# google-deepmind/dm_control

Measured on AMD Instinct MI355X. Metric: env-steps/s (whole node) at batch 4096; max rel qpos error vs CPU, higher is better.
Workload: dtype f32

## Files before the change

dm_control_amd/batch.py:

```python
import ctypes

import numpy as np

from dm_control_amd import _native
from dm_control_amd import mjcf_compiler

OUT = dict(sensor=1 << 0, xpos=1 << 1, xquat=1 << 2, xmat=1 << 3, xipos=1 << 4,
           geom=1 << 5, site=1 << 6, subtree_com=1 << 7, qacc=1 << 8,
           actuator=1 << 9, contact=1 << 10, qfrc=1 << 11, cvel=1 << 12, contact_ids=1 << 13)
OUT_ALL = 0x7fffffff


class BatchedPhysics:

  def __init__(self, model, batch_size, device_id=0, precision=32, nconmax=0,
               njmax=0, lanes_per_env=0, njcon=0, specialise=None):
    if not isinstance(model, mjcf_compiler.Model):
      raise TypeError('model must be a compiled mjcf_compiler.Model')
    L = _native.lib()
    self.model = model
    self.model_real = {}
    self.batch_size = int(batch_size)
    self.precision = precision
    self.device_id = device_id
# ... 34 lines not shown
  def set_task_args(self, blob):
    buf = (ctypes.c_char * len(blob)).from_buffer_copy(blob)
    _native.check(_native.lib().dmc_batch_set_task_args(self._ptr, ctypes.cast(buf, ctypes.c_void_p), len(blob)))

  def enable_task(self, on):
    _native.check(_native.lib().dmc_batch_enable_task(self._ptr, int(bool(on))))

  def close(self):
    L = _native.lib()
    if getattr(self, '_ptr', None):
      L.dmc_batch_destroy(self._ptr)
      self._ptr = None
    if getattr(self, '_model_ptr', None):
      L.dmc_model_destroy(self._model_ptr)
      self._model_ptr = None

  def __del__(self):
    try:
      self.close()
    except Exception:
      pass

  def info(self):
    a = np.zeros(21, dtype=np.int32)
    _native.check(_native.lib().dmc_batch_info(self._ptr, a.ctypes.data))
    keys = ['B', 'precision', 'lanes_per_env', 'waves_per_block', 'envs_per_block',
            'lds_bytes_per_block', 'grid', 'nconmax', 'njmax', 'env_scratch_bytes', 'static_id',
            'jac_kmax', 'table_lds_bytes', 'envs_per_cu', 'njdense', 'njcon', 'stash', 'stash_bytes_per_env',
            'global_scratch_bytes_per_env', 'work_queue', 'slices']
    return dict(zip(keys, (int(x) for x in a)))

  def _rows(self, name):
    rows, is_int = ctypes.c_int(), ctypes.c_int()
    _native.check(_native.lib().dmc_batch_field_rows(self._ptr, name.encode(),
                                                     ctypes.byref(rows), ctypes.byref(is_int)))
    return rows.value, bool(is_int.value)

  def get(self, name):
    rows, is_int = self._rows(name)
    if is_int:
      out = np.zeros((self.batch_size, rows), dtype=np.int32)
      _native.check(_native.lib().dmc_batch_get_int(self._ptr, name.encode(), out.ctypes.data))
    else:
      out = np.zeros((self.batch_size, rows), dtype=np.float64)
      if rows:
        _native.check(_native.lib().dmc_batch_get(self._ptr, name.encode(), out.ctypes.data))
    return out

  def set(self, name, value):
    rows, is_int = self._rows(name)
    if not rows:
      return
    dt = np.int32 if is_int else np.float64
# ... 213 lines not shown
```

dm_control_amd/csrc/dmc_api.hip:

```cpp
#include <hip/hip_runtime.h>
#include <dlfcn.h>

#include <cstdio>
#include <cstdlib>
#include <cstring>
#include <algorithm>
#include <string>
#include <type_traits>
#include <vector>

#include "../../include/dmc_batch.h"
#include "step_kernel.hip.h"
#include "step_tables.h"

namespace dmc {
hipError_t launch_step_f32(const LaunchGeom& g, hipStream_t stream, const StepLayout* d_layout, const StepOpts<float>& o,
                           const int* g_mi, const float* g_mr, const int* g_mc, const StepIO<float>& io, int nstep, int legacy, int mode, int outmask, int nsub);
hipError_t launch_step_f64(const LaunchGeom& g, hipStream_t stream, const StepLayout* d_layout, const StepOpts<double>& o,
                           const int* g_mi, const double* g_mr, const int* g_mc, const StepIO<double>& io, int nstep, int legacy, int mode, int outmask, int nsub);
}

using namespace dmc;

static thread_local std::string g_err;
static int fail(const std::string& msg, int code = -1) { g_err = msg; return code; }
#define HIP_TRY(expr)                                                                        \
  do {                                                                                       \
    hipError_t e_ = (expr);                                                                  \
    if (e_ != hipSuccess) return fail(std::string(#expr) + ": " + hipGetErrorString(e_), -2); \
  } while (0)

struct dmc_model {
  HostModel hm;
};

enum FieldId {
#define X(name, count, flags) F_##name,
  DMC_DATA_REAL_FIELDS(X) DMC_DATA_INT_FIELDS(X)
#undef X
  F_env_geom, F_COUNT
};
struct Field {
// ... 35 lines not shown
  int launched_mask = 0;
  int ndebug = 0;
  void* d_debug = nullptr;
  int* d_debug_i = nullptr;
  long long* d_prof = nullptr;
  size_t elem = 0;
  void* d_stash_r = nullptr; int* d_stash_i = nullptr; int* d_epoch = nullptr; int stash_on = 0; int stash_auto = 0;
  int xfrc_on = 0;
  void* d_ns_A = nullptr;
  int* d_work = nullptr;
  int ncu = 0;
  void* d_kstash = nullptr; int* d_kstash_i = nullptr;
  int *d_cost = nullptr, *d_order = nullptr; int lpt = 0, nitems = 0;
  int* d_prog = nullptr; int max_slices = 0;
  unsigned long long* d_hand = nullptr; int hand_n = 0; int nxcd = 1;
  void* d_gscr = nullptr;
  int* d_trace = nullptr;
  Profiler* prof = nullptr;
  Xfer* xfer = nullptr;
  void* d_probe = nullptr; int probe_geom = 0, probe_cap = 0;
  int trace_launch = 0;
  int* d_rj_i = nullptr; double* d_rj_r = nullptr;
  int* d_eg_slot = nullptr;
  void* spec_so = nullptr; void* spec_launch = nullptr; int spec_features = 0;
  int spec_task_bytes = 0;
  void* d_task_args = nullptr; int task_on = 0;
};

template <class Owner, typename P>
static int dev_alloc(Owner* b, P** ptr, size_t bytes, bool zero, const char* what, const void* init = nullptr) {
  void* p = nullptr;
  hipError_t e = hipMalloc(&p, bytes);
  if (e == hipSuccess && zero) e = hipMemset(p, 0, bytes);
  if (e == hipSuccess && init) e = hipMemcpy(p, init, bytes, hipMemcpyHostToDevice);
  if (e != hipSuccess) { if (p) (void)hipFree(p); return fail(std::string("hipMalloc") + (*what ? " " : "") + what + ": " + hipGetErrorString(e), -2); }
  b->dev_bufs.push_back(p);
  *ptr = (P*)p;
  return 0;
}
template <class Owner, typename P>
static void dev_free(Owner* b, P** ptr) {
  if (!*ptr) return;
  b->dev_bufs.erase(std::find(b->dev_bufs.begin(), b->dev_bufs.end(), (void*)*ptr));
  (void)hipFree(*ptr);
  *ptr = nullptr;
}
template <class Owner>
// ... 330 lines not shown
  if (!b || !so_path) return fail("null argument");
  void* h = dlopen(so_path, RTLD_NOW | RTLD_LOCAL);
  if (!h) return fail(std::string("cannot load ") + so_path + ": " + dlerror());
  typedef const StepLayout* (*layout_t)();
  typedef void (*info_t)(int*);
  layout_t fl = (layout_t)dlsym(h, "dmc_spec_layout");
  info_t fi = (info_t)dlsym(h, "dmc_spec_info");
  void* launch = dlsym(h, "dmc_spec_launch");
  if (!fl || !fi || !launch) { dlclose(h); return fail("not a specialisation plugin (dmc_spec_* symbols missing)"); }
  int info[8]; fi(info);
  if (info[4] != b->precision) { dlclose(h); return fail("the plugin was built for another precision"); }
  const int so = b->precision == 64 ? (int)sizeof(StepOpts<double>) : (int)sizeof(StepOpts<float>);
  const int sio = b->precision == 64 ? (int)sizeof(StepIO<double>) : (int)sizeof(StepIO<float>);
  if (info[0] != (int)sizeof(StepLayout) || info[1] != so || info[2] != sio || info[3] != DMC_MODEL_VERSION || info[7] != (int)sizeof(LaunchGeom)) {
    dlclose(h); return fail("the plugin was built from other sources than this library (struct sizes / model version differ)");
  }
  if (info[5] != b->geom.lpe) { dlclose(h); return fail("the plugin was built for another lanes-per-environment shape"); }
  if (memcmp(fl(), &b->tb.L, sizeof(StepLayout)) != 0) { dlclose(h); return fail("the plugin's layout is not this batch's (another model or other caps)"); }
  if (b->spec_so) dlclose(b->spec_so);
  b->spec_so = h; b->spec_launch = launch; b->spec_features = info[6];
  typedef int (*tb_t)();
  tb_t tb = (tb_t)dlsym(h, "dmc_spec_task_args_bytes");
  b->spec_task_bytes = tb ? tb() : 0;
  b->task_on = 0;
  return bump_epoch(b, 0, true);
}

extern "C" int dmc_batch_set_task_args(dmc_batch* b, const void* args, int nbytes) {
  if (!b || !args) return fail("null argument");
  if (!b->spec_task_bytes) return fail("the batch's kernel carries no task epilogue (attach a plugin built with a task header)");
  if (nbytes != b->spec_task_bytes) return fail("task argument block: size differs from the one the kernel was generated with");
  HIP_TRY(hipSetDevice(b->device));
  if (!b->d_task_args && dev_alloc(b, &b->d_task_args, (size_t)nbytes, false, "task arguments")) return -2;
  HIP_TRY(hipMemcpy(b->d_task_args, args, (size_t)nbytes, hipMemcpyHostToDevice));
  return 0;
}
extern "C" int dmc_batch_enable_task(dmc_batch* b, int on) {
  if (!b) return fail("null batch");
  if (on && (!b->spec_task_bytes || !b->d_task_args)) return fail("no task epilogue to enable (dmc_batch_set_task_args first)");
  b->task_on = on ? 1 : 0;
  return 0;
}

extern "C" int dmc_batch_step(dmc_batch* b, int nstep, int legacy_step, void* hip_stream) {
  if (!b) return fail("null batch");
  if (nstep < 1) return fail("nstep must be >= 1");
// ... 549 lines not shown
    if (reset_real(F_mocap_pos, mp.data(), 3*m.nmocap)) return -2;
    if (reset_real(F_mocap_quat, mq.data(), 4*m.nmocap)) return -2;
  }
  Field* w = &b->fields[F_warning];
  std::vector<int32_t> wh((size_t)B * DMC_NWARNING, 0);
  if (env_mask) { if (get_int(b, w, wh.data())) return -2; for (int e = 0; e < B; e++) if (env_mask[e]) for (int k = 0; k < DMC_NWARNING; k++) wh[(size_t)e * DMC_NWARNING + k] = 0; }
  return set_int(b, w, wh.data());
}

extern "C" int dmc_batch_info(const dmc_batch* b, int* info) {
  if (!b || !info) return fail("null argument");
  const StepLayout& L = b->tb.L;
  info[0] = b->B; info[1] = b->precision; info[2] = b->geom.lpe; info[3] = b->geom.waves; info[4] = b->geom.envs_per_block;
  info[5] = b->geom.lds_bytes; info[6] = b->geom.grid; info[7] = L.d.nconmax; info[8] = L.d.njmax;
  info[9] = (int)((size_t)L.n_sr * b->elem + (size_t)L.n_si * sizeof(int));
  info[10] = b->spec_launch ? 1000 : b->geom.static_id;
  info[11] = L.d.kmax;
  info[12] = b->geom.lds_bytes - b->geom.envs_per_block * info[9];
  { long blocks = (160L * 1024) / b->geom.lds_bytes; if (blocks * b->geom.waves > 8) blocks = 8 / b->geom.waves; info[13] = (int)(blocks * b->geom.envs_per_block); }
  info[14] = L.d.njdense; info[15] = L.d.njcon; info[16] = b->stash_on; info[17] = (int)((size_t)L.n_keep * b->elem + (size_t)(L.n_si + 4) * sizeof(int));
  info[18] = (int)((size_t)L.n_gs * b->elem);
  info[19] = b->geom.queue;
  info[20] = b->geom.queue ? b->max_slices : 0;
  return 0;
}

extern "C" int dmc_batch_enable_profiling(dmc_batch* b, int enabled) {
  if (!b) return fail("null batch");
  if (!b->prof) b->prof = new Profiler();
  b->prof->on = enabled != 0;
  return 0;
}
extern "C" int dmc_batch_get_timer(dmc_batch* b, int timer, double* duration_s, long long* number) {
  if (!b || !duration_s || !number) return fail("null argument");
  if (timer != 0 && timer != 1) return fail("timer must be 0 (mjTIMER_STEP) or 1 (mjTIMER_FORWARD)");
  *duration_s = 0; *number = 0;
  if (!b->prof) return 0;
  HIP_TRY(hipSetDevice(b->device));
  prof_drain(b->prof, true);
  *duration_s = b->prof->duration[timer]; *number = b->prof->number[timer];
  return 0;
}
extern "C" int dmc_batch_time_steps(dmc_batch* b, int nstep, int legacy_step, int reps, void* hip_stream, float* ms_per_launch) {
  if (!b || !ms_per_launch || reps < 1) return fail("bad argument");
  HIP_TRY(hipSetDevice(b->device));
  hipEvent_t e0, e1;
// ... 883 lines not shown
```

dm_control_amd/csrc/ik_kernels.hip:

```cpp
#include <hip/hip_runtime.h>

#include <string>
#include <vector>

#include "../../include/dmc_ik.h"
#include "ik_core.h"

namespace dmc {

constexpr int kIkBlock = 64;
constexpr int kIkLdsBudget = 64*1024;
constexpr int ik_table_bytes(const IkDims& d, int rb) { return (ik_nreals(d)*rb + ik_nints(d)*4 + 15) & ~15; }

template <typename T>
struct IkArgs {
  IkChain<T> ch;
  IkOpts<T> o;
  int B, nq, epb;
  const T* tpos;
  const T* tquat;
  const T* qin;
  long long qin_sk, qin_se;
  T* qbatch;
  T* qout;
// ... 76 lines not shown
  a.ch.reals = static_cast<const T*>(ik->d_reals);
  const dmc_ik_options& o = ik->opt;
  a.o.tol = (T)o.tol; a.o.rot_weight = (T)o.rot_weight; a.o.reg_threshold = (T)o.regularization_threshold;
  a.o.reg_strength = (T)o.regularization_strength; a.o.max_update_norm = (T)o.max_update_norm;
  a.o.progress_thresh = (T)o.progress_thresh; a.o.max_steps = o.max_steps;
  a.B = ik->B; a.nq = ik->nq; a.epb = ik->epb;
  a.tpos = static_cast<const T*>(tpos); a.tquat = static_cast<const T*>(tquat);
  if (qin) { a.qin = static_cast<const T*>(qin); a.qin_sk = 1; a.qin_se = ik->nq; }
  else { a.qin = qbatch; a.qin_sk = ik->B; a.qin_se = 1; }
  a.qbatch = inplace ? qbatch : nullptr;
  a.qout = static_cast<T*>(qout); a.err = static_cast<T*>(err); a.steps = steps; a.status = status;
  const dim3 grid((unsigned)((ik->B + ik->epb - 1)/ik->epb)), block(kIkBlock);
  const size_t lds = (size_t)ik->lds;
  if (tpos && tquat) hipLaunchKernelGGL((ik_kernel<T, IK_BOTH>), grid, block, lds, stream, a);
  else if (tpos) hipLaunchKernelGGL((ik_kernel<T, IK_POS>), grid, block, lds, stream, a);
  else hipLaunchKernelGGL((ik_kernel<T, IK_ROT>), grid, block, lds, stream, a);
  return hipGetLastError() == hipSuccess ? 0 : -2;
}
}

extern "C" int dmc_ik_create(dmc_batch* b, const dmc_ik_chain* c, const dmc_ik_options* opt, dmc_ik** out) {
  if (!b || !c || !opt || !out) return ik_fail("dmc_ik_create: null argument");
  *out = nullptr;
  int info[21] = {0};
  if (dmc_batch_info(b, info) != 0) return ik_fail(std::string("dmc_ik_create: ") + dmc_last_error());
  int nq = 0, is_int = 0;
  if (dmc_batch_field_rows(b, "qpos", &nq, &is_int) != 0 || is_int) return ik_fail("dmc_ik_create: the batch has no qpos");
  IkDims d = {c->nbody, c->njnt, c->ndof, c->nqchain};
  if (d.nb < 1 || d.nj < 1 || d.nd < 1 || d.nqc < 1) return ik_fail("dmc_ik_create: the site's chain has no joint");
  if (d.nd > kIkMaxDof) return ik_fail("dmc_ik_create: " + std::to_string(d.nd) + " chain dofs, at most " + std::to_string(kIkMaxDof));
  if (d.nqc > 2*kIkMaxDof || d.nj > d.nd || d.nb > 4096) return ik_fail("dmc_ik_create: inconsistent chain sizes");
  if (opt->max_steps < 1) return ik_fail("dmc_ik_create: max_steps must be at least 1");
  static const int qw[4] = {7, 4, 1, 1}, dw[4] = {6, 3, 1, 1};
  std::vector<int> rot(d.nd, 0), seen(d.nj, 0);
  int nmov = 0;
  for (int k = 0; k < d.nb; k++) {
    const int j0 = c->body_jntadr[k], jn = c->body_jntnum[k];
    if (jn < 0 || (jn > 0 && (j0 < 0 || j0 + jn > d.nj))) return ik_fail("dmc_ik_create: body joint range outside the chain");
    for (int j = j0; j < j0 + jn; j++) {
      seen[j]++;
      if (c->jnt_type[j] == DMC_JNT_FREE && jn != 1) return ik_fail("dmc_ik_create: a free joint must be its body's only joint");
    }
  }
  for (int j = 0; j < d.nj; j++) {
    const int t = c->jnt_type[j];
    if (seen[j] != 1) return ik_fail("dmc_ik_create: every chain joint must belong to exactly one chain body");
    if (t < 0 || t > 3) return ik_fail("dmc_ik_create: unknown joint type");
// ... 80 lines not shown
```

dm_control_amd/csrc/step_core.h:

```cpp
#pragma once
#include "../../include/dmc_model_layout.h"
#include "step_layout.h"
#include "step_defs.h"
#include "step_math.h"
#include "step_lanes.h"
#include "step_dense.h"
#include "step_geom.h"

namespace dmc {
#ifdef DMC_HOST_EMU
inline int& emu_split_solves() { static int n = 0; return n; }
inline long long* emu_ls_counts() { static long long n[6] = {0, 0, 0, 0, 0, 0}; return n; }
inline long long* emu_ls_passes() { static long long n[3] = {0, 0, 0}; return n; }
#endif

#if defined(DMC_PROFILE) && !defined(DMC_HOST_EMU)
#define DMC_PROF(id) do { if (lane == 0) { const int t_ = (int)__builtin_readcyclecounter(); SI(prof)[id] += t_ - SI(prof)[33]; SI(prof)[33] = t_; } } while (0)
#else
#define DMC_PROF(id) ((void)0)
#endif
#ifdef DMC_TRACE_SUB
#define DMC_TSUB(region, cond, row) do { if (DMC_TRACE_SUB == (region) && (cond)) sub_stamp(row); } while (0)
#else
#define DMC_TSUB(region, cond, row) ((void)0)
// ... 4500 lines not shown
    badv = group_max<LPE>(badv);
    if (badv) { if (lane == 0) SI(imisc)[IM_WARN + DMC_WARN_BADQVEL]++; if (!(o.disableflags & DMC_DSBL_AUTORESET)) { DMC_WSYNC(); reset_state(); } }
    return (badp || badv) && !(o.disableflags & DMC_DSBL_AUTORESET);
  }
  DMC_DEV bool bad_acc() {
    int bad = 0;
    FOR_LANES(i, L.d.nv) if (t_bad(S(qacc)[i])) bad = 1;
    return group_max<LPE>(bad) != 0;
  }

  DMC_DEV void stage_posvel(bool partial, int outmask, bool skipsensor, bool havekin = false) {
    if (!havekin) { kinematics(); DMC_PROF(PROF_KIN); DMC_TSUB(1, partial, 4); com_pos(); DMC_PROF(PROF_COM); DMC_TSUB(1, partial, 5); }
    if (!partial) { crb_mass_matrix(); DMC_PROF(PROF_CRB); DMC_TSUB(2, true, 4); }
    if (!partial || (outmask & (OUT_CONTACT | OUT_CONTACT_IDS))) { collision(); DMC_PROF(PROF_COLL); DMC_TSUB(2, !partial, 5); }
    if (!partial) { make_constraint(); DMC_PROF(PROF_CONSTR); DMC_TSUB(2, true, 6); }
    if (!skipsensor) sensors(DMC_STAGE_POS);
    DMC_PROF(PROF_SENS);
    DMC_TSUB(1, partial, 6);
    if (!havekin) { com_vel(); DMC_PROF(PROF_COMVEL); DMC_TSUB(1, partial, 7); }
    if (!partial) { passive_and_rne(); DMC_PROF(PROF_RNE); DMC_TSUB(2, true, 7); }
    if (!skipsensor) sensors(DMC_STAGE_VEL);
    DMC_PROF(PROF_SENS);
  }
  DMC_DEV void stage_acc(bool disable_actuation, bool skipsensor, bool euler_next = false) {
    fwd_actuation(disable_actuation); DMC_PROF(PROF_ACT);
    bool regs = false;
#ifndef DMC_HOST_EMU
    if constexpr (kAccRegs) {
      const int nefc = SI(imisc)[IM_NEFC];
      if (lane == 0) S(misc)[kMiscEulerSolved] = 0;
      regs = acc_regs_ok(nefc);
      if (regs) {
        const bool damped = euler_next && o.any_damping && !(o.disableflags & (DMC_DSBL_EULERDAMP | DMC_DSBL_DAMPER))
                            && !(kFeat && o.integrator == DMC_INT_IMPLICITFAST);
        primal_solve_regs<LS::kNV, true>(nefc, false, 0, 0, 1, damped);
      }
    }
#endif
    if (!regs) { fwd_acceleration(); DMC_PROF(PROF_ACC); fwd_constraint(); }
    DMC_PROF(PROF_X8);
    if (!skipsensor) sensors_acc();
    DMC_PROF(PROF_SENS);
  }
  DMC_DEV void sub_stamp(int row) {
#if defined(DMC_TRACE_SUB) && !defined(DMC_HOST_EMU)
    const StepIO<T>* iop = (const StepIO<T>*)((const unsigned char*)&o + (sizeof(StepOpts<T>) + 15) / 16 * 16);
// ... 92 lines not shown
    if (stash) store_stash(io, env, false);
    store_state(io, env);
  }
  DMC_DEV TaskLds<T> task_lds() const {
    TaskLds<T> v;
    v.qpos = S(qpos); v.qvel = S(qvel); v.ctrl = S(ctrl); v.act = S(act); v.sensordata = S(sensordata); v.xpos = S(xpos);
    v.xmat = S(xmat); v.xipos = S(xipos); v.subtree_com = S(subtree_com); v.geom_xpos = S(geom_xpos); v.cvel = S(cvel);
    return v;
  }
  DMC_DEV void probe_store(const StepIO<T>& io, int env, int first, int count) {
    if constexpr (!kFeat) return;
    env = late(env);
    T* p = io.probe;
    if (!p) return;
    const int cap = io.probe_cap, g = io.probe_geom;
    for (int t = first; t < first + count && t < cap; t++) FOR_LANES(k, 3) p[((size_t)t*3 + k)*io.B + env] = S(geom_xpos)[3*g + k];
  }
  DMC_DEV void run(const StepIO<T>& io, int env, int nstep, int legacy, int mode, int outmask, int nsub) {
    Entry en; EntryRegs er;
    entry_issue(L, o, io, env, lane, mode, legacy, &en, &er);
    entry_commit(L, io, env, lane, &en, er, s);
    run(io, env, nstep, legacy, mode, outmask, nsub, en);
  }
  DMC_DEV void run(const StepIO<T>& io, int env, int nstep, int legacy, int mode, int outmask, int nsub, const Entry& en,
                   int piece = 0, int npieces = 1) {
    const int launch_mode = mode;
    if (lane == 0) set_epoch(en.epoch);
    if (io.env_mode) {
      const int em = en.em;
      if (em == 2) return;
      if (em == 1 && (mode == 0 || mode >= 4)) mode = 2;
    }
    if constexpr (!kSlices) { piece = 0; npieces = 1; }
    if (mode != 0 && piece != npieces - 1) return;
    if (mode != 0) { piece = 0; npieces = 1; }
    if (mode >= 4) { run_split(io, env, mode, outmask, en); return; }
    prof_begin();
    const bool stash = io.stash_r != nullptr;
    bool have = false;
    if (stash && mode == 0 && legacy && o.integrator != DMC_INT_RK4) have = load_stash(io, env);
    load_state(io, env, have, en, kSlices && piece > 0);
    bool havekin = false;
    if (piece == 0 && io.kstash && mode == 0 && launch_mode == 0 && legacy && !have && o.integrator != DMC_INT_RK4) {
      if (!en.fast) havekin = load_kstash(io, env);
      else if (en.kvalid) { havekin = true; DMC_WSYNC(); kstash_env_geoms(); }
    }
    DMC_PROF(PROF_LOAD);
    const bool stepping = mode == 0 || mode == 3;
    const int ntotal = mode == 3 ? nstep*nsub : nstep;
    const int npass = !stepping ? 1 : ntotal + ((legacy || mode == 3) ? 1 : 0);
    const bool fwd_after = kFeat && legacy == 2 && mode == 0;
    const bool last_piece = piece == npieces - 1;
    const int it_lo = npieces > 1 ? (int)((long long)piece * ntotal / npieces) : 0;
    const int it_hi = (npieces > 1 && !last_piece) ? (int)((long long)(piece + 1) * ntotal / npieces) : npass;
    for (int it = it_lo; it < it_hi; it++) {
      const bool trailing = stepping && it == ntotal;
      const bool partial = trailing && !(stash && mode == 0) && !fwd_after;
      if (mode == 3 && !trailing && it % nsub == 0 && io.ctrl_seq) load_ctrl_seq(io, env, it / nsub);
      if (stepping) { if (check_pos_vel()) { have = false; havekin = false; } }
      const int nstage = (stepping && !trailing && o.integrator == DMC_INT_RK4) ? 4 : 1;
      const bool sens_pv = !stepping || it == npass - 1 || (mode == 3 && it % nsub == 0);
      const bool sens_acc = !stepping || (it == ntotal - 1 && !fwd_after) || (trailing && fwd_after) || (mode == 3 && (it + 1) % nsub == 0);
      int stage = 0, retried = 0;
      while (stage < nstage) {
        if (!(have && it == 0 && !retried)) call_posvel(partial, outmask, stage > 0 || !sens_pv, havekin && it == 0 && !retried && !trailing);
        if (it == 0 && stage == 0) trace_stamp(io, env, 4); else if (trailing) trace_stamp(io, env, 7);
        if (mode == 3 && stage == 0 && it > 0 && it % nsub == 0) store_seq(io, env, it / nsub - 1);
        if (mode == 0 && stage == 0 && it >= 1) probe_store(io, env, it - 1, 1);
        if (trailing && !fwd_after) break;
        call_acc(mode == 2, stage > 0 || !sens_acc, stepping && !trailing && nstage == 1);
        if (trailing) break;
        if (it == 0 && stage == 0) trace_stamp(io, env, 5);
        if (stage == 0 && stepping && !retried && bad_acc()) {
          if (lane == 0) SI(imisc)[IM_WARN + DMC_WARN_BADQACC]++;
          if (!(o.disableflags & DMC_DSBL_AUTORESET)) { DMC_WSYNC(); reset_state(); retried = 1; continue; }
        }
        if (stage == 0 && stepping && it == ntotal - 1) { dump_debug(io, env); if (mode == 0 && !legacy) store_outputs(io, env, outmask); }
        if (nstage > 1) rk4_stage(stage);
        stage++;
      }
      if (!stepping || trailing) break;
      if (nstage > 1) rk4_finish(); else call_euler();
      if (it == 0) trace_stamp(io, env, 6);
      DMC_PROF(PROF_EULER);
    }
    if constexpr (kSlices) if (!last_piece) { store_handoff(io, env); DMC_PROF(PROF_STORE); prof_end(io, env); return; }
    if (!stepping) dump_debug(io, env);
    if (!stepping && launch_mode == 0) probe_store(io, env, 0, nstep);
    if (kWideIO) store_time(io, env);
    if (!stepping || legacy || mode == 3) { DMC_PROF(PROF_TRAIL); store_outputs(io, env, outmask); }
    if (stash) store_stash(io, env, mode == 0 && legacy && !fwd_after);
    if (io.kstash && mode == 0 && legacy && o.integrator != DMC_INT_RK4) store_kstash(io, env);
    store_state(io, env, kWideIO);
    DMC_PROF(PROF_STORE);
    prof_end(io, env);
  }
#undef MI
#undef MR
#undef GC
#undef S
#undef SG
#undef SI
#undef FOR_LANES
};


#ifndef DMC_HOST_EMU
template <typename T, int LPE, typename LS>
struct StageFns {
  typedef StepCore<T, LPE, LS> Core;
  static DMC_FN void posvel(LS ls, const DMC_LDS StepOpts<T>* o, DMC_LDS int* mi, DMC_LDS T* mr, const int* gc, DMC_LDS T* s,
                            DMC_LDS int* si, int lane, int flags, int outmask) {
    Core c(ls, *(const StepOpts<T>*)o, (const int*)mi, (const T*)mr, gc, (T*)s, (int*)si, lane);
    c.stage_posvel(flags & 1, outmask, flags & 2, flags & 4);
  }
  static DMC_FN void acc(LS ls, const DMC_LDS StepOpts<T>* o, DMC_LDS int* mi, DMC_LDS T* mr, const int* gc, DMC_LDS T* s,
                         DMC_LDS int* si, int lane, int flags) {
    Core c(ls, *(const StepOpts<T>*)o, (const int*)mi, (const T*)mr, gc, (T*)s, (int*)si, lane);
    c.stage_acc(flags & 1, flags & 2, flags & 4);
  }
  static DMC_FN void ns_build(LS ls, const DMC_LDS StepOpts<T>* o, DMC_LDS int* mi, DMC_LDS T* mr, const int* gc, DMC_LDS T* s,
                              DMC_LDS int* si, int lane, int nf) {
    if constexpr (LS::kNV > 0 && LS::kNV <= 32 && LPE == 64) {
      Core c(ls, *(const StepOpts<T>*)o, (const int*)mi, (const T*)mr, gc, (T*)s, (int*)si, lane);
      c.template noslip_build_A_lanes<LS::kNV>((const DMC_LDS T*)c.M_factor(), nf, c.row_map());
    }
  }
  static DMC_FN void euler(LS ls, const DMC_LDS StepOpts<T>* o, DMC_LDS int* mi, DMC_LDS T* mr, const int* gc, DMC_LDS T* s,
                           DMC_LDS int* si, int lane) {
    Core c(ls, *(const StepOpts<T>*)o, (const int*)mi, (const T*)mr, gc, (T*)s, (int*)si, lane);
    c.euler_state();
  }
};
#endif

}
```

dm_control_amd/csrc/step_kernel.hip.h:

```cpp
#pragma once
#include <hip/hip_runtime.h>

#include "step_core.h"
#ifdef DMC_TASK_HEADER
#define DMC_TASK_IN_KERNEL 1
#include DMC_TASK_HEADER
#endif

namespace dmc {

struct LaunchGeom {
  int lpe;
  int waves;
  int envs_per_block;
  int lds_bytes;
  int grid;
  int queue;
  int blocks_per_cu;
  int static_id;
};

#ifndef DMC_MIN_WAVES
#define DMC_MIN_WAVES 2
#endif
// ... 3 lines not shown

#if defined(DMC_LAYOUTS_HEADER)
#include DMC_LAYOUTS_HEADER
#elif defined(DMC_PROFILE) && __has_include("static_layouts_prof.gen.h")
#include "static_layouts_prof.gen.h"
#elif __has_include("static_layouts.gen.h")
#include "static_layouts.gen.h"
#endif
#ifndef DMC_NSTATIC
#define DMC_NSTATIC 0
#endif

template <typename T> constexpr int stepopts_lds_bytes() { return (int)((sizeof(StepOpts<T>) + 15) / 16 * 16); }
template <typename T> constexpr int opts_lds_bytes() { return stepopts_lds_bytes<T>() + (int)((sizeof(StepIO<T>) + 15) / 16 * 16); }

#ifndef DMC_NO_WIDE_IO
typedef unsigned int u32x4 __attribute__((ext_vector_type(4)));
#define DMC_KARG __attribute__((address_space(4)))
template <typename T> constexpr int kernarg_io_offset(int karg0) {
  static_assert(alignof(StepOpts<T>) == 8 && alignof(StepIO<T>) == 8 && sizeof(StepOpts<T>) % 8 == 0 && sizeof(StepIO<T>) % 8 == 0, "kernel-argument layout");
  return karg0 + (int)sizeof(StepOpts<T>) + 3 * (int)sizeof(void*);
}
#endif

template <typename T, int LPE, typename LS, bool QUEUE, int KARG0>
__device__ __forceinline__ void step_kernel_body(LS ls, const StepOpts<T>& o_arg, const int* __restrict__ g_mi,
                                                 const T* __restrict__ g_mr, const int* __restrict__ g_mc, const StepIO<T>& io_arg, int nstep, int legacy,
                                                 int mode, int outmask, int nsub) {
  extern __shared__ __attribute__((aligned(16))) unsigned char smem[];
  const StepLayout& L = ls.get();
  StepOpts<T>* o_lds = reinterpret_cast<StepOpts<T>*>(smem);
  unsigned char* tables = smem + opts_lds_bytes<T>();
  int* mi = reinterpret_cast<int*>(tables);
  T* mr = reinterpret_cast<T*>(tables + (size_t)L.n_mi * sizeof(int));
  const int tid = threadIdx.x, nthr = blockDim.x;
  const int t_entry = io_arg.trace ? (int)(wall_clock64() & 0x7fffffffll) : 0;
  typedef StepCore<T, LPE, LS> Core;
  constexpr int epw = 64 / LPE;
  const int nblk = gridDim.x, xcd = blockIdx.x & 7, q = nblk >> 3, r = nblk & 7;
  const int lblk = xcd * q + (xcd < r ? xcd : r) + (blockIdx.x >> 3);
  const int wave = __builtin_amdgcn_readfirstlane(tid >> 6), wpb = nthr >> 6;
  const int nitems = (io_arg.B + epw - 1) / epw, nwaves = nblk * wpb;
  const size_t tables_bytes = (size_t)L.n_mi * sizeof(int) + (size_t)L.n_mr_lds * sizeof(T) + (L.d.coldlds ? (size_t)L.n_mc * sizeof(int) : 0);
  const size_t env_bytes = (size_t)L.n_sr * sizeof(T) + (size_t)L.n_si * sizeof(int);
  typename Core::Entry en;
  typename Core::EntryRegs er;
// ... 11 lines not shown
#pragma unroll
    for (int k = 0; k < arg_trips; k++) {
      areg[k] = 0;
      if (k * nthr < n_arg) {
        int d = tid + k * nthr;
        d = d < n_arg ? d : n_arg - 1;
        areg[k] = *(const DMC_KARG unsigned*)(ka + (d < n_argo ? KARG0 + 4 * d : io_off + 4 * (d - n_argo)));
      }
    }
  }
#endif
  const StepIO<T>& io = *io_lds;
  int* const q_work = QUEUE ? io_arg.work : nullptr;
  int* const q_prog = QUEUE ? io_arg.prog : nullptr;
  const int q_slices = QUEUE ? io_arg.slices : 0, q_nxcd = QUEUE ? io_arg.nxcd : 1;
  const int NX = (QUEUE && q_work && q_nxcd > 1) ? q_nxcd : 1;
  const int xq = NX > 1 ? (int)(__builtin_amdgcn_s_getreg(20 | (0 << 6) | (3 << 11)) % (unsigned)NX) : 0;
  const int nq_items = (nitems - xq + NX - 1) / NX;
  const int npieces = (Core::kSlices && QUEUE && q_work && q_prog && q_slices > 1 && mode == 0) ? q_slices : 1;
  const int nslots = nq_items * npieces;
  int* const head = (QUEUE && q_work) ? q_work + 32 * (1 + xq) : nullptr;
  int slot = lblk * wpb + wave, piece = 0;
  bool have_item = slot < nitems;
  if (QUEUE && head) {
    int nx = 0;
    if ((tid & 63) == 0) nx = atomicAdd(head, 1);
    nx = __builtin_amdgcn_readfirstlane(nx);
    have_item = nx < nslots;
    for (piece = 0; nx >= nq_items && piece < npieces - 1; piece++) nx -= nq_items;
    slot = nx * NX + xq;
  }
  int env0 = 0;
  if (have_item && piece == 0) {
    const int item = io_arg.order ? io_arg.order[slot] : slot;
    env0 = item * epw + ((tid / LPE) & (epw - 1));
    if (env0 >= io_arg.B) env0 = io_arg.B - 1;
    Core::entry_issue(L, o_arg, io_arg, env0, tid % LPE, mode, legacy, &en, &er);
  } else if (have_item) {
    const int item = io_arg.order ? io_arg.order[slot] : slot;
    int e0 = item * epw + ((tid / LPE) & (epw - 1));
    if (e0 >= io_arg.B) e0 = io_arg.B - 1;
    en.em = io_arg.env_mode ? io_arg.env_mode[e0] : 0; en.fast = 0; en.kvalid = 0; en.epoch = *io_arg.epoch;
  }
  int* mc_lds = reinterpret_cast<int*>(tables + (size_t)L.n_mi * sizeof(int) + (size_t)L.n_mr_lds * sizeof(T));
  const size_t cold_bytes = L.d.coldlds ? (size_t)L.n_mc * sizeof(int) : 0;
#ifdef DMC_NO_WIDE_IO
// ... 35 lines not shown
      if (d < n_arg) *reinterpret_cast<unsigned*>(smem + (d < n_argo ? 4 * d : stepopts_lds_bytes<T>() + 4 * (d - n_argo))) = areg[k];
    }
  }
#endif
  if (have_item && piece == 0) Core::entry_commit(L, io_arg, env0, tid % LPE, &en, er, reinterpret_cast<T*>(tables + tables_bytes + (size_t)(tid / LPE) * env_bytes));
  __syncthreads();
  if (have_item) for (;;) {
    int t = threadIdx.x;
    asm volatile("" : "+v"(t));
    const int g = t / LPE, lane = t % LPE;
    unsigned char* base = tables + (size_t)L.n_mi * sizeof(int) + (size_t)L.n_mr_lds * sizeof(T) + cold_bytes + (size_t)g * env_bytes;
    T* s = reinterpret_cast<T*>(base);
    int* si = reinterpret_cast<int*>(base + (size_t)L.n_sr * sizeof(T));
    StepCore<T, LPE, LS> core(ls, *o_lds, mi, mr, L.d.coldlds ? (const int*)mc_lds : g_mc, s, si, lane);
    const int item = io.order ? io.order[slot] : slot;
    const int env = item * epw + (g & (epw - 1));
    int* tr = io.trace ? io.trace + (size_t)(io.trace_slot & 7) * 8 * nitems : nullptr;
    const long long tw0 = tr ? (long long)wall_clock64() : 0;
    if (QUEUE && piece > 0)
      while (__hip_atomic_load(q_prog + item, __ATOMIC_RELAXED, __HIP_MEMORY_SCOPE_AGENT) < piece) __builtin_amdgcn_s_sleep(8);
    const long long tw1 = tr ? (long long)wall_clock64() : 0;
    const long long t0 = io.cost ? (long long)__builtin_readcyclecounter() : 0;
    if (tr && (threadIdx.x & 63) == 0 && piece == 0) { tr[item] = t_entry; tr[nitems + item] = (int)(wall_clock64() & 0x7fffffffll); }
    if (env < io.B) core.run(io, env, nstep, legacy, mode, outmask, nsub, en, piece, npieces);
#ifdef DMC_TASK_HEADER
    if (io.task_args && mode == 0 && piece == npieces - 1 && env < io.B) {
      if (dmc_task::kReadsGlobal) asm volatile("s_waitcnt vmcnt(0)" ::: "memory");
      if (lane == 0) dmc_task::task_post(*(const dmc_task::PostArgs*)io.task_args, env, core.task_lds());
    }
#endif
    if (tr && (threadIdx.x & 63) == 0 && piece == npieces - 1) {
      tr[2*nitems + item] = (int)(wall_clock64() & 0x7fffffffll);
      tr[3*nitems + item] = (int)blockIdx.x;
    }
    if (tr && (threadIdx.x & 63) == 0) {
      const int wt = (int)(tw1 - tw0), rn = (int)((long long)wall_clock64() - tw1);
      if (piece == 0) { __hip_atomic_store(tr + 4*nitems + item, wt, __ATOMIC_RELAXED, __HIP_MEMORY_SCOPE_AGENT); __hip_atomic_store(tr + 5*nitems + item, rn, __ATOMIC_RELAXED, __HIP_MEMORY_SCOPE_AGENT); }
      else { atomicAdd(tr + 4*nitems + item, wt); atomicAdd(tr + 5*nitems + item, rn); }
    }
    if (io.cost && (threadIdx.x & 63) == 0) {
      long long dt = ((long long)__builtin_readcyclecounter() - t0) >> 6;
      dt = dt < 1 ? 1 : (dt > 0x07ffffff ? 0x07ffffff : dt);
      if (piece == 0) __hip_atomic_store(io.cost + item, (int)dt, __ATOMIC_RELAXED, __HIP_MEMORY_SCOPE_AGENT);
      else atomicAdd(io.cost + item, (int)dt);
    }
    if (QUEUE && piece < npieces - 1) {
      asm volatile("s_waitcnt vmcnt(0)" ::: "memory");
      if ((threadIdx.x & 63) == 0) __hip_atomic_store(q_prog + item, piece + 1, __ATOMIC_RELAXED, __HIP_MEMORY_SCOPE_AGENT);
    }
    if (!QUEUE || !head) break;
    int nx = 0;
    if ((threadIdx.x & 63) == 0) nx = atomicAdd(head, 1);
    nx = __builtin_amdgcn_readfirstlane(nx);
    if (nx >= nslots) break;
    for (piece = 0; nx >= nq_items && piece < npieces - 1; piece++) nx -= nq_items;
    slot = nx * NX + xq;
    const int nitem = io.order ? io.order[slot] : slot;
    int nenv = nitem * epw + ((threadIdx.x / LPE) & (epw - 1));
    if (nenv >= io.B) nenv = io.B - 1;
    en.em = io.env_mode ? io.env_mode[nenv] : 0; en.fast = 0; en.kvalid = 0;
  }
  if (QUEUE && q_work && (threadIdx.x & 63) == 0) {
    if (atomicAdd(q_work + 1, 1) == nwaves - 1) {
      atomicExch(q_work + 1, 0);
      for (int x = 0; x < NX; x++) atomicExch(q_work + 32 * (1 + x), 0);
      if (npieces > 1) for (int i = 0; i < nitems; i++) q_prog[i] = 0;
    }
  }
}

template <typename T, int LPE, bool QUEUE>
__global__ void __launch_bounds__(DMC_MAX_THREADS, DMC_MIN_WAVES)
step_kernel(const StepLayout* __restrict__ Lp, StepOpts<T> o, const int* __restrict__ g_mi, const T* __restrict__ g_mr,
            const int* __restrict__ g_mc, StepIO<T> io, int nstep, int legacy, int mode, int outmask, int nsub) {
  DynLayoutSrc ls; ls.p = Lp;
  step_kernel_body<T, LPE, DynLayoutSrc, QUEUE, (int)sizeof(const StepLayout*)>(ls, o, g_mi, g_mr, g_mc, io, nstep, legacy, mode, outmask, nsub);
}

#if DMC_NSTATIC > 0
template <int SID> struct StaticLayout;
#define DMC_DEF_STATIC(ID)                                                            \
  static __device__ const StepLayout kStaticLayout##ID = DMC_STATIC_LAYOUT_##ID;     \
  template <> struct StaticLayout<ID> {                                               \
// ... 47 lines not shown
#else
#define DMC_UNIT_INSTANCES(X) DMC_STATIC_INSTANCES(X)
#endif
  const bool need_feat = legacy == 2 || io.probe != nullptr || o.integrator == DMC_INT_IMPLICITFAST;
#define DMC_X(SID, LPE) if (g.static_id == SID && g.lpe == LPE && (DMC_STATIC_FEATURES || !need_feat)) DMC_LAUNCH_STATIC(LPE, SID)
  DMC_UNIT_INSTANCES(DMC_X)
#undef DMC_X
#endif
#if defined(DMC_UNIT_ILP)
  return hipErrorInvalidValue;
#else
  if (g.lpe == 64) DMC_LAUNCH(64)
  else if (g.lpe == 32) DMC_LAUNCH(32)
  else if (g.lpe == 16) DMC_LAUNCH(16)
  else return hipErrorInvalidValue;
#endif
#undef DMC_LAUNCH
#undef DMC_LAUNCH_STATIC
#undef DMC_LAUNCH_Q
#undef DMC_LAUNCH_STATIC_Q
  return hipGetLastError();
}

}
```

dm_control_amd/csrc/step_kernel_spec.hip:

```cpp
#define DMC_UNIT_ILP 1
#include "step_kernel.hip.h"
using namespace dmc;

#if DMC_SPEC_PRECISION == 64
typedef double spec_real;
#else
typedef float spec_real;
#endif

extern "C" const StepLayout* dmc_spec_layout() { static const StepLayout L = DMC_STATIC_LAYOUT_0; return &L; }
extern "C" void dmc_spec_info(int* out) {
  out[0] = (int)sizeof(StepLayout); out[1] = (int)sizeof(StepOpts<spec_real>); out[2] = (int)sizeof(StepIO<spec_real>);
  out[3] = DMC_MODEL_VERSION; out[4] = DMC_SPEC_PRECISION; out[5] = DMC_SPEC_LPE; out[6] = DMC_STATIC_FEATURES; out[7] = (int)sizeof(LaunchGeom);
}
extern "C" int dmc_spec_launch(const LaunchGeom* g, void* stream, const StepLayout* d_layout, const StepOpts<spec_real>* o,
                               const int* g_mi, const spec_real* g_mr, const int* g_mc, const StepIO<spec_real>* io, int nstep,
                               int legacy, int mode, int outmask, int nsub) {
  LaunchGeom gg = *g;
  gg.static_id = 0;
  return (int)launch_step_t<spec_real>(gg, (hipStream_t)stream, d_layout, *o, g_mi, g_mr, g_mc, *io, nstep, legacy, mode, outmask, nsub);
}
#ifdef DMC_TASK_HEADER
extern "C" int dmc_spec_task_args_bytes() { return (int)sizeof(dmc_task::PostArgs); }
#endif
```

dm_control_amd/csrc/step_kernels_f32.hip:

```cpp
#define DMC_UNIT_STD 1
#define DMC_STATIC_FEATURES 0
#include "step_kernel.hip.h"
namespace dmc {
hipError_t launch_step_f32_ilp(const LaunchGeom& g, hipStream_t stream, const StepLayout* d_layout, const StepOpts<float>& o,
                               const int* g_mi, const float* g_mr, const int* g_mc, const StepIO<float>& io, int nstep, int legacy, int mode, int outmask, int nsub);
hipError_t launch_step_f32(const LaunchGeom& g, hipStream_t stream, const StepLayout* d_layout, const StepOpts<float>& o,
                           const int* g_mi, const float* g_mr, const int* g_mc, const StepIO<float>& io, int nstep, int legacy, int mode, int outmask, int nsub) {
#if DMC_NSTATIC > 0
#define DMC_X(SID, LPE) if (g.static_id == SID && g.lpe == LPE) return launch_step_f32_ilp(g, stream, d_layout, o, g_mi, g_mr, g_mc, io, nstep, legacy, mode, outmask, nsub);
  DMC_STATIC_INSTANCES_ILP(DMC_X)
#undef DMC_X
#endif
  return launch_step_t<float>(g, stream, d_layout, o, g_mi, g_mr, g_mc, io, nstep, legacy, mode, outmask, nsub);
}
}
```

Measured before the change: 82.66 million.

## Split the first step's mass matrix and collision across wave pairs

Adds a cooperative opening phase for 32-lane-per-env f32 kernels. A prelude loads state and checks it. Then the wave pairs in each block split the first step's work across 16-lane rows: one wave runs the CRB mass matrix and passive/RNE while the other runs collision and constraint construction. The main run then resumes and skips posvel on iteration zero. This aims to overlap two independent stages of the opening step, at the cost of extra block-wide barriers, a new code path tied to specific conditions (kstash fast path, no queue, even wave count), and a reporting field in info().

```diff
diff --git a/dm_control_amd/batch.py b/dm_control_amd/batch.py
--- a/dm_control_amd/batch.py
+++ b/dm_control_amd/batch.py
@@ -80,13 +80,15 @@
       pass
 
   def info(self):
-    a = np.zeros(21, dtype=np.int32)
+    a = np.zeros(22, dtype=np.int32)
     _native.check(_native.lib().dmc_batch_info(self._ptr, a.ctypes.data))
     keys = ['B', 'precision', 'lanes_per_env', 'waves_per_block', 'envs_per_block',
             'lds_bytes_per_block', 'grid', 'nconmax', 'njmax', 'env_scratch_bytes', 'static_id',
             'jac_kmax', 'table_lds_bytes', 'envs_per_cu', 'njdense', 'njcon', 'stash', 'stash_bytes_per_env',
             'global_scratch_bytes_per_env', 'work_queue', 'slices']
-    return dict(zip(keys, (int(x) for x in a)))
+    out = dict(zip(keys, (int(x) for x in a)))
+    out['launch'] = {'coop_open': int(a[21])}
+    return out
 
   def _rows(self, name):
     rows, is_int = ctypes.c_int(), ctypes.c_int()
diff --git a/dm_control_amd/csrc/dmc_api.hip b/dm_control_amd/csrc/dmc_api.hip
--- a/dm_control_amd/csrc/dmc_api.hip
+++ b/dm_control_amd/csrc/dmc_api.hip
@@ -18,6 +18,7 @@
                            const int* g_mi, const float* g_mr, const int* g_mc, const StepIO<float>& io, int nstep, int legacy, int mode, int outmask, int nsub);
 hipError_t launch_step_f64(const LaunchGeom& g, hipStream_t stream, const StepLayout* d_layout, const StepOpts<double>& o,
                            const int* g_mi, const double* g_mr, const int* g_mc, const StepIO<double>& io, int nstep, int legacy, int mode, int outmask, int nsub);
+int step_coop_open_f32(const LaunchGeom& g);
 }
 
 using namespace dmc;
@@ -99,7 +100,7 @@
   int trace_launch = 0;
   int* d_rj_i = nullptr; double* d_rj_r = nullptr;
   int* d_eg_slot = nullptr;
-  void* spec_so = nullptr; void* spec_launch = nullptr; int spec_features = 0;
+  void* spec_so = nullptr; void* spec_launch = nullptr; int spec_features = 0; int spec_coop = 0;
   int spec_task_bytes = 0;
   void* d_task_args = nullptr; int task_on = 0;
 };
@@ -476,6 +477,8 @@
   typedef int (*tb_t)();
   tb_t tb = (tb_t)dlsym(h, "dmc_spec_task_args_bytes");
   b->spec_task_bytes = tb ? tb() : 0;
+  tb_t fc = (tb_t)dlsym(h, "dmc_spec_coop_open");
+  b->spec_coop = fc ? fc() : 0;
   b->task_on = 0;
   return bump_epoch(b, 0, true);
 }
@@ -1071,6 +1074,8 @@
   info[18] = (int)((size_t)L.n_gs * b->elem);
   info[19] = b->geom.queue;
   info[20] = b->geom.queue ? b->max_slices : 0;
+  const int coop_kernel = b->spec_launch ? b->spec_coop : (b->precision == 32 ? step_coop_open_f32(b->geom) : 0);
+  info[21] = (coop_kernel && b->geom.waves % 2 == 0 && !b->geom.queue && b->d_kstash && !b->stash_on) ? 1 : 0;
   return 0;
 }
 
diff --git a/dm_control_amd/csrc/ik_kernels.hip b/dm_control_amd/csrc/ik_kernels.hip
--- a/dm_control_amd/csrc/ik_kernels.hip
+++ b/dm_control_amd/csrc/ik_kernels.hip
@@ -122,7 +122,7 @@
 extern "C" int dmc_ik_create(dmc_batch* b, const dmc_ik_chain* c, const dmc_ik_options* opt, dmc_ik** out) {
   if (!b || !c || !opt || !out) return ik_fail("dmc_ik_create: null argument");
   *out = nullptr;
-  int info[21] = {0};
+  int info[22] = {0};
   if (dmc_batch_info(b, info) != 0) return ik_fail(std::string("dmc_ik_create: ") + dmc_last_error());
   int nq = 0, is_int = 0;
   if (dmc_batch_field_rows(b, "qpos", &nq, &is_int) != 0 || is_int) return ik_fail("dmc_ik_create: the batch has no qpos");
diff --git a/dm_control_amd/csrc/step_core.h b/dm_control_amd/csrc/step_core.h
--- a/dm_control_amd/csrc/step_core.h
+++ b/dm_control_amd/csrc/step_core.h
@@ -4546,6 +4546,23 @@
     if (!skipsensor) sensors(DMC_STAGE_VEL);
     DMC_PROF(PROF_SENS);
   }
+  DMC_DEV void coop_side_a() { crb_mass_matrix(); passive_and_rne(); }
+  DMC_DEV void coop_side_b() { collision(); make_constraint(); }
+  static constexpr int kMiscCoop = 3, kCoopOpened = 1, kCoopEntered = 2;
+#if !defined(DMC_HOST_EMU) && !defined(DMC_NO_COOP_OPEN) && !defined(DMC_PROFILE) && !defined(DMC_TRACE_SUB)
+  static constexpr bool kCoopOpen = kAccRegs && LPE == 32;
+#else
+  static constexpr bool kCoopOpen = false;
+#endif
+  DMC_DEV int coop_prelude(const StepIO<T>& io, int env, int nstep, int legacy, int mode, const Entry& en) {
+    if (io.env_mode && en.em != 0) return 0;
+    if (!(mode == 0 && nstep >= 1 && legacy && io.kstash && !io.stash_r && o.integrator != DMC_INT_RK4 && en.fast && en.kvalid)) return 0;
+    if (lane == 0) set_epoch(en.epoch);
+    load_state(io, env, false, en);
+    DMC_WSYNC();
+    kstash_env_geoms();
+    return check_pos_vel() ? kCoopEntered : (kCoopEntered | kCoopOpened);
+  }
   DMC_DEV void stage_acc(bool disable_actuation, bool skipsensor, bool euler_next = false) {
     fwd_actuation(disable_actuation); DMC_PROF(PROF_ACT);
     bool regs = false;
@@ -4684,29 +4701,36 @@
     entry_commit(L, io, env, lane, &en, er, s);
     run(io, env, nstep, legacy, mode, outmask, nsub, en);
   }
-  DMC_DEV void run(const StepIO<T>& io, int env, int nstep, int legacy, int mode, int outmask, int nsub, const Entry& en,
-                   int piece = 0, int npieces = 1) {
+  DMC_DEV int run(const StepIO<T>& io, int env, int nstep, int legacy, int mode, int outmask, int nsub, const Entry& en,
+                  int piece = 0, int npieces = 1, int ph = 0) {
     const int launch_mode = mode;
-    if (lane == 0) set_epoch(en.epoch);
+    int cst = 0;
+    if constexpr (kCoopOpen) {
+      if (ph == 1) return coop_prelude(io, env, nstep, legacy, mode, en);
+      if (ph == 2) cst = (int)S(misc)[kMiscCoop];
+    }
+    const bool resumed = kCoopOpen && (cst & kCoopEntered);
+    if (!resumed) { if (lane == 0) set_epoch(en.epoch); }
     if (io.env_mode) {
       const int em = en.em;
-      if (em == 2) return;
+      if (em == 2) return 0;
       if (em == 1 && (mode == 0 || mode >= 4)) mode = 2;
     }
     if constexpr (!kSlices) { piece = 0; npieces = 1; }
-    if (mode != 0 && piece != npieces - 1) return;
+    if (mode != 0 && piece != npieces - 1) return 0;
     if (mode != 0) { piece = 0; npieces = 1; }
-    if (mode >= 4) { run_split(io, env, mode, outmask, en); return; }
+    if (mode >= 4) { run_split(io, env, mode, outmask, en); return 0; }
     prof_begin();
     const bool stash = io.stash_r != nullptr;
     bool have = false;
     if (stash && mode == 0 && legacy && o.integrator != DMC_INT_RK4) have = load_stash(io, env);
-    load_state(io, env, have, en, kSlices && piece > 0);
+    if (!resumed) load_state(io, env, have, en, kSlices && piece > 0);
     bool havekin = false;
-    if (piece == 0 && io.kstash && mode == 0 && launch_mode == 0 && legacy && !have && o.integrator != DMC_INT_RK4) {
+    if (!resumed && piece == 0 && io.kstash && mode == 0 && launch_mode == 0 && legacy && !have && o.integrator != DMC_INT_RK4) {
       if (!en.fast) havekin = load_kstash(io, env);
       else if (en.kvalid) { havekin = true; DMC_WSYNC(); kstash_env_geoms(); }
     }
+    const bool opened = resumed && (cst & kCoopOpened);
     DMC_PROF(PROF_LOAD);
     const bool stepping = mode == 0 || mode == 3;
     const int ntotal = mode == 3 ? nstep*nsub : nstep;
@@ -4719,13 +4743,13 @@
       const bool trailing = stepping && it == ntotal;
       const bool partial = trailing && !(stash && mode == 0) && !fwd_after;
       if (mode == 3 && !trailing && it % nsub == 0 && io.ctrl_seq) load_ctrl_seq(io, env, it / nsub);
-      if (stepping) { if (check_pos_vel()) { have = false; havekin = false; } }
+      if (stepping && !(resumed && it == 0)) { if (check_pos_vel()) { have = false; havekin = false; } }
       const int nstage = (stepping && !trailing && o.integrator == DMC_INT_RK4) ? 4 : 1;
       const bool sens_pv = !stepping || it == npass - 1 || (mode == 3 && it % nsub == 0);
       const bool sens_acc = !stepping || (it == ntotal - 1 && !fwd_after) || (trailing && fwd_after) || (mode == 3 && (it + 1) % nsub == 0);
       int stage = 0, retried = 0;
       while (stage < nstage) {
-        if (!(have && it == 0 && !retried)) call_posvel(partial, outmask, stage > 0 || !sens_pv, havekin && it == 0 && !retried && !trailing);
+        if (!((have || opened) && it == 0 && !retried)) call_posvel(partial, outmask, stage > 0 || !sens_pv, havekin && it == 0 && !retried && !trailing);
         if (it == 0 && stage == 0) trace_stamp(io, env, 4); else if (trailing) trace_stamp(io, env, 7);
         if (mode == 3 && stage == 0 && it > 0 && it % nsub == 0) store_seq(io, env, it / nsub - 1);
         if (mode == 0 && stage == 0 && it >= 1) probe_store(io, env, it - 1, 1);
@@ -4746,7 +4770,7 @@
       if (it == 0) trace_stamp(io, env, 6);
       DMC_PROF(PROF_EULER);
     }
-    if constexpr (kSlices) if (!last_piece) { store_handoff(io, env); DMC_PROF(PROF_STORE); prof_end(io, env); return; }
+    if constexpr (kSlices) if (!last_piece) { store_handoff(io, env); DMC_PROF(PROF_STORE); prof_end(io, env); return 0; }
     if (!stepping) dump_debug(io, env);
     if (!stepping && launch_mode == 0) probe_store(io, env, 0, nstep);
     if (kWideIO) store_time(io, env);
@@ -4756,6 +4780,7 @@
     store_state(io, env, kWideIO);
     DMC_PROF(PROF_STORE);
     prof_end(io, env);
+    return 0;
   }
 #undef MI
 #undef MR
@@ -4776,6 +4801,17 @@
     Core c(ls, *(const StepOpts<T>*)o, (const int*)mi, (const T*)mr, gc, (T*)s, (int*)si, lane);
     c.stage_posvel(flags & 1, outmask, flags & 2, flags & 4);
   }
+  typedef StepCore<T, 16, LS> Core16;
+  static DMC_FN void coop_a(LS ls, const DMC_LDS StepOpts<T>* o, DMC_LDS int* mi, DMC_LDS T* mr, const int* gc, DMC_LDS T* s,
+                            DMC_LDS int* si, int lane, int on) {
+    Core16 c(ls, *(const StepOpts<T>*)o, (const int*)mi, (const T*)mr, gc, (T*)s, (int*)si, lane);
+    if (on) c.coop_side_a();
+  }
+  static DMC_FN void coop_b(LS ls, const DMC_LDS StepOpts<T>* o, DMC_LDS int* mi, DMC_LDS T* mr, const int* gc, DMC_LDS T* s,
+                            DMC_LDS int* si, int lane, int on) {
+    Core16 c(ls, *(const StepOpts<T>*)o, (const int*)mi, (const T*)mr, gc, (T*)s, (int*)si, lane);
+    if (on) c.coop_side_b();
+  }
   static DMC_FN void acc(LS ls, const DMC_LDS StepOpts<T>* o, DMC_LDS int* mi, DMC_LDS T* mr, const int* gc, DMC_LDS T* s,
                          DMC_LDS int* si, int lane, int flags) {
     Core c(ls, *(const StepOpts<T>*)o, (const int*)mi, (const T*)mr, gc, (T*)s, (int*)si, lane);
diff --git a/dm_control_amd/csrc/step_kernel.hip.h b/dm_control_amd/csrc/step_kernel.hip.h
--- a/dm_control_amd/csrc/step_kernel.hip.h
+++ b/dm_control_amd/csrc/step_kernel.hip.h
@@ -49,6 +49,32 @@
   return karg0 + (int)sizeof(StepOpts<T>) + 3 * (int)sizeof(void*);
 }
 #endif
+
+template <typename T, int LPE, typename LS>
+__device__ __forceinline__ void coop_open_phase(LS ls, const StepOpts<T>* o_lds, int* mi, T* mr, const int* gc, unsigned char* envs,
+                                                size_t env_bytes, int st) {
+  typedef StepCore<T, LPE, LS> Core;
+  static_assert(LPE == 32, "a wave pair holds four environments, a wave four 16-lane rows");
+  const StepLayout& L = ls.get();
+  int t = threadIdx.x;
+  asm volatile("" : "+v"(t));
+  if (t % LPE == 0) reinterpret_cast<T*>(envs + (size_t)(t / LPE) * env_bytes)[L.s_misc + Core::kMiscCoop] = (T)st;
+  __syncthreads();
+  {
+    const int slot = ((t >> 6) & ~1) * (64 / LPE) + ((t & 63) >> 4);
+    unsigned char* base = envs + (size_t)slot * env_bytes;
+    T* s = reinterpret_cast<T*>(base);
+    int* si = reinterpret_cast<int*>(base + (size_t)L.n_sr * sizeof(T));
+    const int on = (int)s[L.s_misc + Core::kMiscCoop] & Core::kCoopOpened;
+    if (__builtin_amdgcn_ballot_w64(on != 0)) {
+      if (__builtin_amdgcn_readfirstlane(t >> 6) & 1)
+        StageFns<T, LPE, LS>::coop_b(ls, (const DMC_LDS StepOpts<T>*)o_lds, (DMC_LDS int*)mi, (DMC_LDS T*)mr, gc, (DMC_LDS T*)s, (DMC_LDS int*)si, t & 15, on);
+      else
+        StageFns<T, LPE, LS>::coop_a(ls, (const DMC_LDS StepOpts<T>*)o_lds, (DMC_LDS int*)mi, (DMC_LDS T*)mr, gc, (DMC_LDS T*)s, (DMC_LDS int*)si, t & 15, on);
+    }
+  }
+  __syncthreads();
+}
 
 template <typename T, int LPE, typename LS, bool QUEUE, int KARG0>
 __device__ __forceinline__ void step_kernel_body(LS ls, const StepOpts<T>& o_arg, const int* __restrict__ g_mi,
@@ -106,6 +132,8 @@
   int* const head = (QUEUE && q_work) ? q_work + 32 * (1 + xq) : nullptr;
   int slot = lblk * wpb + wave, piece = 0;
   bool have_item = slot < nitems;
+  const bool coop = Core::kCoopOpen && !QUEUE && (nthr & 127) == 0 && mode == 0 && legacy && nstep >= 1 && io_arg.kstash && !io_arg.stash_r;
+  (void)coop;
   if (QUEUE && head) {
     int nx = 0;
     if ((tid & 63) == 0) nx = atomicAdd(head, 1);
@@ -187,7 +215,16 @@
     const long long tw1 = tr ? (long long)wall_clock64() : 0;
     const long long t0 = io.cost ? (long long)__builtin_readcyclecounter() : 0;
     if (tr && (threadIdx.x & 63) == 0 && piece == 0) { tr[item] = t_entry; tr[nitems + item] = (int)(wall_clock64() & 0x7fffffffll); }
-    if (env < io.B) core.run(io, env, nstep, legacy, mode, outmask, nsub, en, piece, npieces);
+    if constexpr (Core::kCoopOpen && !QUEUE) {
+      if (coop) {
+        int st = 0;
+        if (env < io.B) st = core.run(io, env, nstep, legacy, mode, outmask, nsub, en, piece, npieces, 1);
+        coop_open_phase<T, LPE, LS>(ls, o_lds, mi, mr, L.d.coldlds ? (const int*)mc_lds : g_mc, tables + tables_bytes, env_bytes, st);
+      }
+      if (env < io.B) core.run(io, env, nstep, legacy, mode, outmask, nsub, en, piece, npieces, coop ? 2 : 0);
+    } else {
+      if (env < io.B) core.run(io, env, nstep, legacy, mode, outmask, nsub, en, piece, npieces);
+    }
 #ifdef DMC_TASK_HEADER
     if (io.task_args && mode == 0 && piece == npieces - 1 && env < io.B) {
       if (dmc_task::kReadsGlobal) asm volatile("s_waitcnt vmcnt(0)" ::: "memory");
@@ -224,6 +261,8 @@
     int nenv = nitem * epw + ((threadIdx.x / LPE) & (epw - 1));
     if (nenv >= io.B) nenv = io.B - 1;
     en.em = io.env_mode ? io.env_mode[nenv] : 0; en.fast = 0; en.kvalid = 0;
+  } else if constexpr (Core::kCoopOpen && !QUEUE) {
+    if (coop) coop_open_phase<T, LPE, LS>(ls, o_lds, mi, mr, L.d.coldlds ? (const int*)mc_lds : g_mc, tables + tables_bytes, env_bytes, 0);
   }
   if (QUEUE && q_work && (threadIdx.x & 63) == 0) {
     if (atomicAdd(q_work + 1, 1) == nwaves - 1) {
@@ -317,4 +356,15 @@
   return hipGetLastError();
 }
 
-}
+template <typename T>
+static int step_kernel_coop_open(const LaunchGeom& g) {
+#if DMC_NSTATIC > 0
+#define DMC_X(SID, LPE) if (g.static_id == SID && g.lpe == LPE) return StepCore<T, LPE, StaticLayout<SID>>::kCoopOpen ? 1 : 0;
+  DMC_UNIT_INSTANCES(DMC_X)
+#undef DMC_X
+#endif
+  (void)g;
+  return 0;
+}
+
+}
diff --git a/dm_control_amd/csrc/step_kernel_spec.hip b/dm_control_amd/csrc/step_kernel_spec.hip
--- a/dm_control_amd/csrc/step_kernel_spec.hip
+++ b/dm_control_amd/csrc/step_kernel_spec.hip
@@ -20,6 +20,11 @@
   gg.static_id = 0;
   return (int)launch_step_t<spec_real>(gg, (hipStream_t)stream, d_layout, *o, g_mi, g_mr, g_mc, *io, nstep, legacy, mode, outmask, nsub);
 }
+extern "C" int dmc_spec_coop_open() {
+  LaunchGeom g = {};
+  g.static_id = 0; g.lpe = DMC_SPEC_LPE;
+  return step_kernel_coop_open<spec_real>(g);
+}
 #ifdef DMC_TASK_HEADER
 extern "C" int dmc_spec_task_args_bytes() { return (int)sizeof(dmc_task::PostArgs); }
 #endif
diff --git a/dm_control_amd/csrc/step_kernels_f32.hip b/dm_control_amd/csrc/step_kernels_f32.hip
--- a/dm_control_amd/csrc/step_kernels_f32.hip
+++ b/dm_control_amd/csrc/step_kernels_f32.hip
@@ -13,4 +13,5 @@
 #endif
   return launch_step_t<float>(g, stream, d_layout, o, g_mi, g_mr, g_mc, io, nstep, legacy, mode, outmask, nsub);
 }
+int step_coop_open_f32(const LaunchGeom& g) { return step_kernel_coop_open<float>(g); }
 }
```

Measured after the change: 86.45 million, median of 6. 1.05x the previous value.
